# yxlao/deepSpeech

Hardware: AMD Instinct MI355X
Metric: audio-sec/sec training throughput (whole node), DS2 BiGRU (higher is better)
Workload: dtype bf16; 1 GPU; model=DeepSpeech2 2xconv(32) + 5xBiGRU-800 bidirectional + CTC, global_batch=32, seq_len=1000, parallelism=dp1, engine=hip

## Files before the change

### deepspeech_amd/csrc/api.h

```cpp
#pragma once
#include <hip/hip_runtime_api.h>
#include <stddef.h>

extern "C" {

struct DS2Fill {
  int n;
  unsigned* ptr[8];
  unsigned long long words[8];
  unsigned pattern[8];
};

hipEvent_t ds2_take_stop_event();
void ds2_arm_stop_event(hipEvent_t e);

int ds2_multi_fill(int n, void* const* ptrs, const unsigned long long* bytes, const unsigned* patterns,
                   hipStream_t st);
int ds2_multi_copy(int n, void* const* dst, const void* const* src, const unsigned long long* rows,
                   const unsigned* src_row, const unsigned* dst_row, const unsigned* src_pitch,
                   const unsigned* dst_pitch, float* sdst, const float* svals, int ns, hipStream_t st);
int ds2_wait_resident(const unsigned* word, long long timeout, hipStream_t st);
int ds2_prep_inputs(const float* x, void* y, long long n, const int* lens_in, int* lens_out, int nl,
                    hipStream_t st);
int ds2_transpose_bf16(const void* in, void* out, int R, int C, int ldi, int ldo, hipStream_t st);
// ... 205 lines not shown
                     int W, unsigned seed_lo, unsigned seed_hi, unsigned step_lo, unsigned step_hi,
                     unsigned first_utt, hipStream_t st);
int ds2_specaug_mean(const float* x, const int* lens, float* mean, int B, int T, int F, hipStream_t st);
int ds2_specaug_apply(const float* x, const int* lens, const int* plan, const float* mean, float* out, int B, int T,
                      int F, int nF, int nT, int inplace, hipStream_t st);

int ds2_seq_dropout(const void* x, void* out, const int* ctr, int T, int N, int H, unsigned seed_lo,
                    unsigned seed_hi, int site, int thr, float scale, int locked, hipStream_t st);

struct DS2Conv1WgradBn {
  const void *dz, *y1;
  const float *mean, *invstd, *gamma, *beta, *dbeta, *dgamma;
};

struct DS2Conv2DgradBn {
  const void* y1;
  const float *mean, *invstd, *gamma, *beta;
  float* part;
};

size_t ds2_conv2_fwd_smem(int F1);
size_t ds2_conv2_dgrad_smem(int F2);
size_t ds2_conv2_wgrad_smem(int F1);
long long ds2_conv2_wgrad_part_floats(int grid);
long long ds2_conv1_wgrad_part_floats(int grid);
int ds2_conv1_fwd_grid(int N, int T1);
int ds2_conv1_fwd(const void* x, const void* w, const float* bias, void* y, float* part, int N, int T, int F0,
                  int T1, int F1, hipStream_t st);
int ds2_conv2_fwd(const void* x, const void* w, const float* bias, void* y, float* part, int grid, int N, int T1,
                  int F1, int T2, int F2, long long* trace, hipStream_t st);
int ds2_conv2_dgrad(const void* dy, const void* w, void* dx, int grid, int N, int T1, int F1, int T2, int F2,
                    const DS2Conv2DgradBn* bn, long long* trace, hipStream_t st);
int ds2_conv2_wgrad(const void* dy, const void* x, float* part, int grid, float* dw, int N, int T1, int F1, int T2,
                    int F2, hipStream_t st);
int ds2_conv1_wgrad(const void* dy, const void* x, float* part, int grid, float* dw, int N, int T, int F0, int T1,
                    int F1, const DS2Conv1WgradBn* bn, hipStream_t st);
int ds2_bn_cl_finalize(const float* part, int nb, double M, float eps, float* mean, float* invstd, float* run_mean,
                       float* run_var, float momentum, hipStream_t st);
int ds2_bn_cl_apply(const void* y, const float* mean, const float* invstd, const float* gamma, const float* beta,
                    void* out, int N, int T, int F, int tmaj, hipStream_t st);
int ds2_bn_cl_bwd(const void* dz, const void* y, const float* mean, const float* invstd, const float* gamma,
                  const float* beta, float* part, int nb, float* dgamma, float* dbeta, void* dy, int N, int T, int F,
                  int tmaj, int part_ready, hipStream_t st);

struct DS2Feat {
  const void* pcm;
  long long row_stride;
  int S, lead, mode, B, T_max;
  const int* lens;
  const float* offset;
  const float* gain;
  const float* basis;
  const int* mel_idx;
  const float* mel_w;
  const float* dct;
  const float* lifter;
  void* out;
  int* frames;
};

int ds2_audio_stats(const void* pcm, int in_i16, long long row_stride, int S, int B, const int* lens, float* offset,
                    float* gain, hipStream_t st);
int ds2_featurize(const DS2Feat* a, int kind, int in_i16, int out_bf16, hipStream_t st);

}
```

### deepspeech_amd/csrc/bindings.cpp

```cpp
#include <torch/extension.h>
#include <c10/hip/HIPStream.h>
#include <hip/hip_runtime.h>

#include <cstdint>
#include <string>
#include <vector>

#include "api.h"

namespace {

using OptT = c10::optional<at::Tensor>;

hipStream_t cur_stream() { return c10::hip::getCurrentHIPStream().stream(); }

void check(int rc, const char* what) {
  TORCH_CHECK(rc == 0, "deepspeech_amd kernel launch failed in ", what, " (code ", rc, ")");
}

constexpr unsigned kLightEvent = hipEventDisableTiming;

int64_t event_new(unsigned flags) {
  hipEvent_t e = nullptr;
  TORCH_CHECK(hipEventCreateWithFlags(&e, flags ? flags : kLightEvent) == hipSuccess, "hipEventCreateWithFlags");
// ... 474 lines not shown
  need_bf16(x, "x"); need_bf16(w, "w"); need_bf16(y, "y");
  TORCH_CHECK(x.dim() == 4 && y.dim() == 4 && x.size(3) == 32 && y.size(3) == 32 && w.numel() == 32 * 32 * 50,
              "conv2_fwd shapes");
  TORCH_CHECK(grid > 0, "grid");
  need_f32(part, "part", grid * 64);
  check(ds2_conv2_fwd(x.data_ptr(), w.data_ptr(), ptr_or_null<float>(bias, "bias"), y.data_ptr(),
                      part.data_ptr<float>(), (int)grid, (int)x.size(0), (int)x.size(1), (int)x.size(2),
                      (int)y.size(1), (int)y.size(2), trace_ptr(trace), cur_stream()), "conv2_fwd");
}

void conv2_dgrad(at::Tensor dy, at::Tensor w, at::Tensor dx, int64_t grid, OptT y1, OptT mean, OptT invstd,
                 OptT gamma, OptT beta, OptT part, OptT trace) {
  need_bf16(dy, "dy"); need_bf16(w, "w"); need_bf16(dx, "dx");
  TORCH_CHECK(dy.dim() == 4 && dx.dim() == 4 && dy.size(3) == 32 && dx.size(3) == 32 && w.numel() == 32 * 32 * 50,
              "conv2_dgrad shapes");
  TORCH_CHECK(grid > 0, "grid");
  DS2Conv2DgradBn bn{};
  const bool with_bn = y1.has_value();
  if (with_bn) {
    TORCH_CHECK(mean && invstd && gamma && beta && part, "conv2_dgrad: the BN arguments come all or none");
    need_bf16(*y1, "y1");
    TORCH_CHECK(y1->sizes() == dx.sizes(), "y1 must have dx's shape");
    need_f32(*mean, "mean", 32); need_f32(*invstd, "invstd", 32); need_f32(*gamma, "gamma", 32);
    need_f32(*beta, "beta", 32); need_f32(*part, "part", grid * 64);
    bn = DS2Conv2DgradBn{y1->data_ptr(), mean->data_ptr<float>(), invstd->data_ptr<float>(),
                         gamma->data_ptr<float>(), beta->data_ptr<float>(), part->data_ptr<float>()};
  }
  check(ds2_conv2_dgrad(dy.data_ptr(), w.data_ptr(), dx.data_ptr(), (int)grid, (int)dx.size(0), (int)dx.size(1),
                        (int)dx.size(2), (int)dy.size(1), (int)dy.size(2), with_bn ? &bn : nullptr,
                        trace_ptr(trace), cur_stream()),
        "conv2_dgrad");
}

void conv2_wgrad(at::Tensor dy, at::Tensor x, at::Tensor part, at::Tensor dw, int64_t grid) {
  need_bf16(dy, "dy"); need_bf16(x, "x");
  TORCH_CHECK(grid > 0, "grid");
  need_f32(part, "part", ds2_conv2_wgrad_part_floats((int)grid));
  need_f32(dw, "dw", 32 * 32 * 50);
  check(ds2_conv2_wgrad(dy.data_ptr(), x.data_ptr(), part.data_ptr<float>(), (int)grid, dw.data_ptr<float>(),
                        (int)x.size(0), (int)x.size(1), (int)x.size(2), (int)dy.size(1), (int)dy.size(2),
                        cur_stream()), "conv2_wgrad");
}

void conv1_wgrad(at::Tensor dy, at::Tensor x, at::Tensor part, at::Tensor dw, int64_t grid, OptT y1, OptT mean,
                 OptT invstd, OptT gamma, OptT beta, OptT dbeta, OptT dgamma) {
  need_bf16(dy, "dy"); need_bf16(x, "x");
  TORCH_CHECK(grid > 0, "grid");
  need_f32(part, "part", ds2_conv1_wgrad_part_floats((int)grid));
  need_f32(dw, "dw", 32 * 100);
  DS2Conv1WgradBn bn{};
  const bool with_bn = y1.has_value();
  if (with_bn) {
    TORCH_CHECK(mean && invstd && gamma && beta && dbeta && dgamma, "conv1_wgrad: the BN arguments come all or none");
    need_bf16(*y1, "y1");
    TORCH_CHECK(y1->sizes() == dy.sizes(), "y1 must have dz's shape");
    for (const OptT* t : {&mean, &invstd, &gamma, &beta, &dbeta, &dgamma}) need_f32(**t, "bn vector", 32);
    bn = DS2Conv1WgradBn{dy.data_ptr(), y1->data_ptr(), mean->data_ptr<float>(), invstd->data_ptr<float>(),
                         gamma->data_ptr<float>(), beta->data_ptr<float>(), dbeta->data_ptr<float>(),
                         dgamma->data_ptr<float>()};
  }
  check(ds2_conv1_wgrad(with_bn ? nullptr : dy.data_ptr(), x.data_ptr(), part.data_ptr<float>(), (int)grid,
                        dw.data_ptr<float>(), (int)x.size(0), (int)x.size(1), (int)x.size(2), (int)dy.size(1),
                        (int)dy.size(2), with_bn ? &bn : nullptr, cur_stream()), "conv1_wgrad");
}
int64_t conv2_wgrad_part_floats(int64_t grid) { return ds2_conv2_wgrad_part_floats((int)grid); }
int64_t conv1_wgrad_part_floats(int64_t grid) { return ds2_conv1_wgrad_part_floats((int)grid); }

void bn_cl_finalize(at::Tensor part, int64_t nb, double M, double eps, at::Tensor mean, at::Tensor invstd,
                    OptT run_mean, OptT run_var, double momentum) {
  need_f32(part, "part", nb * 64);
  need_f32(mean, "mean", 32); need_f32(invstd, "invstd", 32);
  check(ds2_bn_cl_finalize(part.data_ptr<float>(), (int)nb, M, (float)eps, mean.data_ptr<float>(),
                           invstd.data_ptr<float>(), ptr_or_null<float>(run_mean, "run_mean"),
                           ptr_or_null<float>(run_var, "run_var"), (float)momentum, cur_stream()), "bn_cl_finalize");
// ... 875 lines not shown
        py::arg("alpha") = 1.0, py::arg("alpha_dev") = py::none(), py::arg("alpha_dev2") = py::none(),
        py::arg("a_col") = false, py::arg("b_col") = false, py::arg("splits") = 1, py::arg("ws") = py::none(),
        py::arg("cnt") = py::none(), py::arg("max_grid") = 0, py::arg("fill") = std::vector<at::Tensor>{},
        py::arg("fill_pat") = std::vector<int64_t>{}, py::arg("ext_red") = false);
  m.def("gemm8_group", &gemm8_group, py::arg("A"), py::arg("B"), py::arg("C"), py::arg("epi"), py::arg("splits"),
        py::arg("a_col"), py::arg("b_col"), py::arg("ws"), py::arg("cnt"), py::arg("max_grid"));
  m.def("gemm8_splits", [](int64_t K, bool fp8, int64_t S) { return ds2_gemm8_splits((int)K, fp8 ? 1 : 0, (int)S); });
  m.def("multi_fill", &multi_fill);
  m.def("col_sum", &col_sum);
  m.def("wait_resident", &wait_resident);
  m.def("fc_bias_grad", &fc_bias_grad);
  m.def("ctc_beam", &ctc_beam);
  m.def("ctc_beam_backtrack", &ctc_beam_backtrack);
  m.def("ctc_beam_lm", &ctc_beam_lm);
  m.def("ctc_beam_backtrack_lm", &ctc_beam_backtrack_lm);
  m.def("event_new", &event_new, py::arg("flags") = 0);
  m.def("arm_stop_event", &arm_stop_event);
  m.def("disarm_stop_event", &disarm_stop_event);
  m.def("event_free", &event_free);
  m.def("event_record", &event_record);
  m.def("event_wait", &event_wait);
  m.def("event_query", &event_query);
  m.def("stream_wait", &stream_wait);
  m.def("ctc_greedy", &ctc_greedy, py::arg("logits"), py::arg("lens"), py::arg("labels"), py::arg("counts"),
        py::arg("blank"), py::arg("score") = py::none());
  m.def("conv1_fwd", &conv1_fwd);
  m.def("conv1_fwd_grid", &conv1_fwd_grid);
  m.def("conv2_fwd", &conv2_fwd, py::arg("x"), py::arg("w"), py::arg("bias"), py::arg("y"), py::arg("part"),
        py::arg("grid"), py::arg("trace") = py::none());
  m.def("conv2_dgrad", &conv2_dgrad, py::arg("dy"), py::arg("w"), py::arg("dx"), py::arg("grid"),
        py::arg("y1") = py::none(), py::arg("mean") = py::none(), py::arg("invstd") = py::none(),
        py::arg("gamma") = py::none(), py::arg("beta") = py::none(), py::arg("part") = py::none(),
        py::arg("trace") = py::none());
  m.def("conv2_wgrad", &conv2_wgrad);
  m.def("conv1_wgrad", &conv1_wgrad, py::arg("dy"), py::arg("x"), py::arg("part"), py::arg("dw"), py::arg("grid"),
        py::arg("y1") = py::none(), py::arg("mean") = py::none(), py::arg("invstd") = py::none(),
        py::arg("gamma") = py::none(), py::arg("beta") = py::none(), py::arg("dbeta") = py::none(),
        py::arg("dgamma") = py::none());
  m.def("conv2_wgrad_part_floats", &conv2_wgrad_part_floats);
  m.def("conv1_wgrad_part_floats", &conv1_wgrad_part_floats);
  m.def("bn_cl_finalize", &bn_cl_finalize);
  m.def("bn_cl_apply", &bn_cl_apply);
  m.def("bn_cl_bwd", &bn_cl_bwd, py::arg("dz"), py::arg("y"), py::arg("mean"), py::arg("invstd"), py::arg("gamma"),
        py::arg("beta"), py::arg("part"), py::arg("nb"), py::arg("dgamma"), py::arg("dbeta"), py::arg("dy"),
        py::arg("tmaj"), py::arg("part_ready") = 0);
  m.def("gemm", &gemm, py::arg("A"), py::arg("B"), py::arg("C"), py::arg("bias"), py::arg("M"), py::arg("N"),
        py::arg("K"), py::arg("a_col"), py::arg("b_col"), py::arg("epi"), py::arg("alpha"), py::arg("cfg"),
        py::arg("alpha_dev") = py::none(), py::arg("Ml") = 0, py::arg("Nl") = 0, py::arg("Kl") = 0,
        py::arg("fill") = std::vector<at::Tensor>{}, py::arg("fill_pat") = std::vector<int64_t>{});
  m.def("gemm_tile", &gemm_tile);
  m.def("head_ctc", &head_ctc, py::arg("h"), py::arg("W"), py::arg("bias"), py::arg("lens"), py::arg("labels"),
        py::arg("label_lens"), py::arg("loss"), py::arg("G"), py::arg("ws"), py::arg("blank"), py::arg("zero_inf"),
        py::arg("mean") = py::none(), py::arg("counter") = py::none(), py::arg("first_bad") = py::none());
  m.def("fc_logits", &fc_logits);
  m.def("lookahead", &lookahead);
  m.def("lookahead_wgrad_parts", &lookahead_wgrad_parts);
  m.def("lookahead_wgrad", &lookahead_wgrad);
  m.def("lookahead_stream", &lookahead_stream);
  m.def("specaug_plan", &specaug_plan);
  m.def("specaug_mean", &specaug_mean);
  m.def("specaug_apply", &specaug_apply, py::arg("x"), py::arg("lens"), py::arg("plan"), py::arg("fill"),
        py::arg("out"), py::arg("nF"), py::arg("nT"), py::arg("inplace"));
  m.def("seq_dropout", &seq_dropout, py::arg("x"), py::arg("out"), py::arg("ctr"), py::arg("seed_lo"),
        py::arg("seed_hi"), py::arg("site"), py::arg("thr"), py::arg("scale"), py::arg("locked"));
  m.def("audio_stats", &audio_stats, py::arg("pcm"), py::arg("lens"), py::arg("offset"), py::arg("gain"));
  m.def("featurize", &featurize, py::arg("pcm"), py::arg("lens"), py::arg("offset"), py::arg("gain"),
        py::arg("basis"), py::arg("mel_idx"), py::arg("mel_w"), py::arg("dct"), py::arg("lifter"), py::arg("kind"),
// ... 13 lines not shown
```

### deepspeech_amd/csrc/conv_frontend.hip

```cpp
#include "common.h"

using namespace ds2;

namespace {

typedef __attribute__((ext_vector_type(16))) float f32x16;
typedef __attribute__((ext_vector_type(4))) short s16x4;
typedef __attribute__((address_space(3))) void lds_void_t;
typedef __attribute__((address_space(3))) s16x4 lds_s16x4_t;

constexpr int CC = 32;
constexpr float CLIP = 20.0f;
constexpr int MT = 3;

__device__ __forceinline__ f32x16 mfma32(bf16x8 a, bf16x8 b, f32x16 c) {
  return __builtin_amdgcn_mfma_f32_32x32x16_bf16(a, b, c, 0, 0, 0);
}

__device__ __forceinline__ void glds16(const void* g, void* lds_wave_base) {
  __builtin_amdgcn_global_load_lds(g, (lds_void_t*)lds_wave_base, 16, 0, 0);
}

__device__ __forceinline__ unsigned swz(unsigned R, unsigned c) { return R * 64u + ((c ^ ((R >> 2) & 3u)) << 4); }

// ... 182 lines not shown
          ssum += vb;
          ssq += vb * vb;
        }
      }
    lds_barrier();
    {
      i32x4* dst = (i32x4*)(a.y + ((size_t)n * a.T2 + t2) * a.F2 * CC);
      for (int q = tid; q < a.F2 * 4; q += 256) dst[q] = ((const i32x4*)stg)[q];
    }
    c2_stamp(a.trace, it, 4);
    lds_barrier();
    if (tile + per < t_hi) issue(tile + per);
    c2_stamp(a.trace, it, 5);
  }
  __syncthreads();
  write_stats(ssum, ssq, (float*)red, 4, a.part);
}

struct Conv2Dgrad {
  const bf16_t* dy;
  const bf16_t* w;
  bf16_t* dx;
  int N, T1, F1, T2, F2;
  const bf16_t* y1;
  const float *mean, *invstd, *gamma, *beta;
  float* part;
  long long* trace;
};
constexpr int C2D_KPW = 25;
constexpr int C2D_PR = 4 + 32 * MT;
constexpr int C2D_BUF = 5 * C2D_PR * PR;
constexpr int C2D_RED = 4 * 6 * 64 * 16;
constexpr int C2D_ROW = 80 * 64;
constexpr int C2D_SMEM = C2D_BUF + C2D_RED + 2 * C2D_ROW;
static_assert(C2D_SMEM >= 16 * CC * C2_KT * C2_KF * 2, "one co half of the weights is staged through LDS");

template <int W>
__device__ __forceinline__ void conv2_dgrad_body(const Conv2Dgrad& a);

__global__ __launch_bounds__(256) __attribute__((amdgpu_waves_per_eu(2, 2))) void conv2_dgrad_kernel(Conv2Dgrad a) {
  DS2_DCHECK(a.F2 <= 32 * MT - 4 && a.F1 == a.F2 + 4 && a.F1 > 64 && a.F1 <= 80);
  switch (uni(threadIdx.x >> 6)) {
    case 0: conv2_dgrad_body<0>(a); break;
    case 1: conv2_dgrad_body<1>(a); break;
    case 2: conv2_dgrad_body<2>(a); break;
    default: conv2_dgrad_body<3>(a); break;
  }
}

template <int W>
__device__ __forceinline__ void conv2_dgrad_body(const Conv2Dgrad& a) {
  extern __shared__ __attribute__((aligned(16))) unsigned char smem[];
  constexpr int w = W, par = W & 1, kh = W >> 1, S0 = kh * C2D_KPW;
  const int tid = threadIdx.x, lane = tid & 63;
  const int hi = lane >> 5, col = lane & 31;
  unsigned char* const buf = smem;
  f32x4* red = (f32x4*)(smem + C2D_BUF);
  unsigned short* stg = (unsigned short*)(smem + C2D_BUF + C2D_RED + par * C2D_ROW);

  bf16x8 bfr[C2D_KPW];
  {
    const unsigned short* wl = (const unsigned short*)smem;
    for (int hh = 0; hh < 2; ++hh) {
      const i32x4* src = (const i32x4*)(a.w + (size_t)hh * 16 * CC * C2_KT * C2_KF);
      for (int o = tid; o < 16 * CC * C2_KT * C2_KF / 8; o += 256) ((i32x4*)smem)[o] = src[o];
      __syncthreads();
#pragma unroll
// ... 6 lines not shown
          bfr[i][j] = (short)wl[(((8 * hi + j) * CC + col) * C2_KT + 2 * ai + par) * C2_KF + kf];
      }
      __syncthreads();
    }
  }
  for (int o = tid * 16; o < C2D_BUF; o += 256 * 16) *(i32x4*)(buf + o) = (i32x4){0, 0, 0, 0};

  const int U = (a.T1 + 1) >> 1;
  const int ntiles = a.N * U;
  const int F2 = a.F2, nq = 5 * F2;
  const int X = (gridDim.x % 8 == 0) ? 8 : 1;
  const int per = (int)gridDim.x / X, xi = (int)blockIdx.x % X, wi = (int)blockIdx.x / X;
  const int t_lo = (int)((long long)ntiles * xi / X), t_hi = (int)((long long)ntiles * (xi + 1) / X);

  auto issue = [&](int t) {
    const int n = t / U, u = t - n * U;
    const bf16_t* base = a.dy + (size_t)n * a.T2 * F2 * CC;
#pragma unroll
    for (int i = 0; i < 8; ++i) {
      const int k = w + 4 * i;
      if (k < 30) {
        const int j = k / 6, r = k % 6;
        const int q = 64 * r + lane;
        if (q < nq) {
          const int pos = (q * 52429) >> 18, c = min(q - 5 * pos, 3);
          const int row = min(max(u - 4 + j, 0), a.T2 - 1);
          glds16(base + ((size_t)row * F2 + pos) * CC + c * 8, buf + (j * C2D_PR + 4) * PR + 1024 * r);
        }
      }
    }
  };
  const unsigned char* const lbase = buf + col * PR + hi * 16;
  const bool bn = a.mean != nullptr;
  const float bmu = bn ? a.mean[col] : 0.f, bis = bn ? a.invstd[col] : 0.f;
  const float bg = bn ? a.gamma[col] : 0.f, bbt = bn ? a.beta[col] : 0.f;
  float bs = 0.f, bq = 0.f;
  auto ldA = [&](int i, bf16x8 (&dst)[MT]) {
    const int s = S0 + i;
    const int ai = s / 10, kf = (s % 10) >> 1;
    const int off = ((4 - ai) * C2D_PR + 4 - kf) * PR + (s & 1) * 32;
#pragma unroll
    for (int m = 0; m < MT; ++m) dst[m] = *(const bf16x8*)(lbase + off + m * 32 * PR);
  };

  __syncthreads();
  int it = 0;
  if (t_lo + wi < t_hi) issue(t_lo + wi);
  for (int tile = t_lo + wi; tile < t_hi; tile += per, ++it) {
    const int n = tile / U, u = tile - n * U;
    c2_stamp(a.trace, it, 0);
    asm volatile("s_waitcnt vmcnt(0)" ::: "memory");
    __syncthreads();
    c2_stamp(a.trace, it, 1);
    f32x16 acc[MT];
#pragma unroll
    for (int m = 0; m < MT; ++m) acc[m] = (f32x16){};
    bf16x8 af[2][MT];
    ldA(0, af[0]);
#pragma unroll
    for (int i = 0; i < C2D_KPW; ++i) {
      if (i + 1 < C2D_KPW) ldA(i + 1, af[(i + 1) & 1]);
      const int t2 = u - (S0 + i) / 10;
      if (t2 >= 0 && t2 < a.T2) {
#pragma unroll
        for (int m = 0; m < MT; ++m) acc[m] = mfma32(af[i & 1][m], bfr[i], acc[m]);
      }
    }
    c2_stamp(a.trace, it, 2);
    lds_barrier();
#pragma unroll
    for (int m = 0; m < MT; ++m)
#pragma unroll
      for (int j = 0; j < 2; ++j) {
        const int g = 2 * (1 - kh) + j;
        red[((w * MT + m) * 2 + j) * 64 + lane] = (f32x4){acc[m][4 * g], acc[m][4 * g + 1], acc[m][4 * g + 2], acc[m][4 * g + 3]};
      }
    lds_barrier();
    f32x4 own[MT][2];
#pragma unroll
    for (int m = 0; m < MT; ++m)
#pragma unroll
      for (int j = 0; j < 2; ++j) {
        const int g = 2 * kh + j;
        own[m][j] = (f32x4){acc[m][4 * g], acc[m][4 * g + 1], acc[m][4 * g + 2], acc[m][4 * g + 3]} +
                    red[(((w ^ 2) * MT + m) * 2 + j) * 64 + lane];
      }
    c2_stamp(a.trace, it, 3);
    const int t1 = 2 * u + par;
    const bool out = t1 < a.T1;
    const size_t rowoff = ((size_t)n * a.T1 + t1) * a.F1 * CC;
    if (out) {
      unsigned short yv[MT][2][4];
      if (bn) {
        const unsigned short* yb = (const unsigned short*)a.y1 + rowoff + 4 * hi * CC + col;
        const int lastoff = (a.F1 - 1 - 4 * hi) * CC;
#pragma unroll
        for (int m = 0; m < MT; ++m)
#pragma unroll
          for (int j = 0; j < 2; ++j)
#pragma unroll
            for (int e = 0; e < 4; ++e) {
              const int fo = (32 * m + 8 * (2 * kh + j) + e) * CC;
              yv[m][j][e] = m < 2 ? yb[fo] : yb[min(fo, lastoff)];
            }
      }
#pragma unroll
      for (int m = 0; m < MT; ++m)
#pragma unroll
        for (int j = 0; j < 2; ++j)
#pragma unroll
          for (int e = 0; e < 4; ++e) {
            const int f1 = 32 * m + 8 * (2 * kh + j) + 4 * hi + e;
            if (m < 2 || f1 < a.F1) {
              const bf16_t d = f2bf(own[m][j][e]);
              stg[f1 * CC + col] = d;
              if (bn) {
                const float xh = (bf2f(yv[m][j][e]) - bmu) * bis;
                const float zz = xh * bg + bbt;
                const float dd = (zz > 0.f && zz < CLIP) ? bf2f(d) : 0.f;
                bs += dd;
                bq += dd * xh;
              }
            }
          }
    }
    lds_barrier();
    if (out) {
      i32x4* dst = (i32x4*)(a.dx + rowoff);
      for (int q = kh * 64 + lane; q < a.F1 * 4; q += 128) dst[q] = ((const i32x4*)stg)[q];
    }
    c2_stamp(a.trace, it, 4);
    if (tile + per < t_hi) issue(tile + per);
    c2_stamp(a.trace, it, 5);
  }
  if (bn) {
    bs += __shfl_xor(bs, 32, 64);
    bq += __shfl_xor(bq, 32, 64);
    float* sh = (float*)red;
    __syncthreads();
    if (lane < 32) { sh[(w * 32 + lane) * 2] = bs; sh[(w * 32 + lane) * 2 + 1] = bq; }
    __syncthreads();
    if (tid < 64) a.part[(size_t)blockIdx.x * 64 + tid] = sh[tid] + sh[64 + tid] + sh[128 + tid] + sh[192 + tid];
  }
}

struct Conv2Wgrad {
  const bf16_t* dy;
  const bf16_t* x;
  float* part;
  int N, T1, F1, T2, F2;
};
constexpr int C2W_PAIRS = C2_KT * C2_KF;
constexpr int C2W_WAVES = 8;
constexpr int C2W_PPW = 7;

__global__ __launch_bounds__(512) void conv2_wgrad_kernel(Conv2Wgrad a) {
  extern __shared__ __attribute__((aligned(16))) unsigned char smem[];
  const int tid = threadIdx.x, lane = tid & 63, w = uni(tid >> 6);
  const int dyBytes = 80 * 64;
  const int xBytes = (9 * a.F1 + 84) * 64;
  const int bufBytes = dyBytes + xBytes;
  unsigned char* const buf0 = smem;
  unsigned char* const buf1 = smem + bufBytes;
  for (int b = 0; b < 2; ++b) {
    unsigned char* bb = b ? buf1 : buf0;
    for (int o = a.F2 * 64 + tid * 4; o < dyBytes; o += 512 * 4) *(unsigned*)(bb + o) = 0u;
    for (int o = 10 * a.F1 * 64 + tid * 4; o < xBytes; o += 512 * 4) *(unsigned*)(bb + dyBytes + o) = 0u;
  }
  const int ntiles = a.N * a.T2;
  const int dyChunks = a.F2 * 4, xChunks = 10 * a.F1 * 4;
  auto issue = [&](int t, unsigned char* dst) {
    const int n = t / a.T2, t2 = t - n * a.T2;
    const unsigned char* sdy = (const unsigned char*)(a.dy + ((size_t)n * a.T2 + t2) * a.F2 * CC);
    const unsigned char* sx = (const unsigned char*)(a.x + ((size_t)n * a.T1 + 2 * t2) * a.F1 * CC);
    for (int p0 = w * 64; p0 < dyChunks; p0 += 512) {
      const int p = p0 + lane;
      if (p < dyChunks) glds16(sdy + (size_t)p * 16, dst + (size_t)p0 * 16);
    }
    for (int p0 = w * 64; p0 < xChunks; p0 += 512) {
      const int p = p0 + lane;
      if (p < xChunks) glds16(sx + (size_t)p * 16, dst + dyBytes + (size_t)p0 * 16);
    }
  };
  const int g = lane >> 4, h = g >> 1, cb = (g & 1) * 16, q = (lane & 15) >> 2, pp = lane & 3;
  const unsigned lofs = (unsigned)((8 * h + q) * 64 + (cb + 4 * pp) * 2);
  const int npairs = (w < C2W_PAIRS - 6 * C2W_WAVES) ? 7 : 6;

  f32x16 acc[C2W_PPW];
#pragma unroll
  for (int i = 0; i < C2W_PPW; ++i) acc[i] = (f32x16){};
  __syncthreads();
  int it = 0;
  if ((int)blockIdx.x < ntiles) issue(blockIdx.x, buf0);
  for (int tile = blockIdx.x; tile < ntiles; tile += gridDim.x, ++it) {
    const unsigned char* cur = (it & 1) ? buf1 : buf0;
    asm volatile("s_waitcnt vmcnt(0)" ::: "memory");
    __syncthreads();
    if (tile + (int)gridDim.x < ntiles) issue(tile + gridDim.x, (it & 1) ? buf0 : buf1);
    const unsigned char* xs = cur + dyBytes;
#pragma unroll
    for (int kk = 0; kk < 5; ++kk) {
      const unsigned k0 = (unsigned)(16 * kk) * 64u;
      const bf16x8 av = cat8(tr_read(cur + k0 + lofs), tr_read(cur + k0 + lofs + 4 * 64));
#pragma unroll
      for (int i = 0; i < C2W_PPW; ++i) {
        if (i < npairs) {
          const int P = w + C2W_WAVES * i;
          const int kt = P / 5, kf = P - 5 * (P / 5);
          const unsigned rb = (unsigned)(kt * a.F1 + kf) * 64u + k0 + lofs;
          const bf16x8 bv = cat8(tr_read(xs + rb), tr_read(xs + rb + 4 * 64));
          acc[i] = mfma32(av, bv, acc[i]);
        }
      }
    }
  }
  f32x4* out = (f32x4*)(a.part + (size_t)blockIdx.x * C2W_PAIRS * 1024);
#pragma unroll
  for (int i = 0; i < C2W_PPW; ++i) {
    if (i < npairs) {
      const int P = w + C2W_WAVES * i;
#pragma unroll
      for (int r4 = 0; r4 < 4; ++r4)
        out[(P * 4 + r4) * 64 + lane] = (f32x4){acc[i][4 * r4], acc[i][4 * r4 + 1], acc[i][4 * r4 + 2], acc[i][4 * r4 + 3]};
    }
  }
}

template <int KIND>
__global__ __launch_bounds__(256) void wgrad_reduce_kernel(const float* __restrict__ part, int nb, int E,
                                                           float* __restrict__ dw) {
  __shared__ f32x4 sh[4][64];
  const int tid = threadIdx.x, g = tid >> 6, l = tid & 63;
  const int e4 = blockIdx.x * 64 + l, E4 = E >> 2;
  const f32x4* p4 = (const f32x4*)part;
  f32x4 s0 = {}, s1 = {};
  int b = g;
  for (; b + 4 < nb; b += 8) {
    s0 += p4[(size_t)b * E4 + e4];
    s1 += p4[(size_t)(b + 4) * E4 + e4];
  }
  if (b < nb) s0 += p4[(size_t)b * E4 + e4];
  sh[g][l] = s0 + s1;
  __syncthreads();
  if (g != 0) return;
  const f32x4 v = sh[0][l] + sh[1][l] + sh[2][l] + sh[3][l];
#pragma unroll
// ... 434 lines not shown
  const long long total = (long long)N * T * F * 4, step = (long long)gridDim.x * 256;
  const bf16x8* y8 = (const bf16x8*)y;
  const bf16x8* d8 = (const bf16x8*)dz;
  bf16x8* o8 = (bf16x8*)dy;
  long long e = (long long)blockIdx.x * 256 + tid;
  for (; e + 3 * step < total; e += 4 * step) {
    bf16x8 v[4], d[4];
#pragma unroll
    for (int k = 0; k < 4; ++k) { v[k] = y8[e + k * step]; d[k] = d8[e + k * step]; }
#pragma unroll
    for (int k = 0; k < 4; ++k) o8[e + k * step] = one(v[k], d[k]);
  }
  for (; e < total; e += step) o8[e] = one(y8[e], d8[e]);
}

template <typename K>
int set_smem(K kernel, size_t bytes) {
  return (int)hipFuncSetAttribute(reinterpret_cast<const void*>(kernel), hipFuncAttributeMaxDynamicSharedMemorySize,
                                  (int)bytes);
}

int shape_ok(int T1, int F1, int T2, int F2) {
  if (F1 < 5 || F1 > 80 || F2 != F1 - 4) return -40;
  if (T1 < 10 || T2 != (T1 - 10) / 2 + 1) return -41;
  return 0;
}

}

extern "C" {

size_t ds2_conv2_fwd_smem(int) { return (size_t)C2F_SMEM; }
size_t ds2_conv2_dgrad_smem(int) { return (size_t)C2D_SMEM; }
size_t ds2_conv2_wgrad_smem(int F1) { return (size_t)2 * (80 * 64 + (9 * F1 + 84) * 64); }
long long ds2_conv2_wgrad_part_floats(int grid) { return (long long)grid * C2W_PAIRS * 1024; }
long long ds2_conv1_wgrad_part_floats(int grid) { return (long long)grid * 5 * 1024; }
int ds2_conv1_fwd_grid(int N, int T1) { return N * ((T1 + C1_ROWS - 1) / C1_ROWS); }

int ds2_conv2_fwd(const void* x, const void* w, const float* bias, void* y, float* part, int grid, int N, int T1,
                  int F1, int T2, int F2, long long* trace, hipStream_t st) {
  if (int e = shape_ok(T1, F1, T2, F2)) return e;
  const size_t smem = ds2_conv2_fwd_smem(F1);
  DS2_HIP_CHECK((hipError_t)set_smem(conv2_fwd_kernel, smem));
  Conv2Fwd a{(const bf16_t*)x, (const bf16_t*)w, bias, (bf16_t*)y, part, N, T1, F1, T2, F2, trace};
  hipLaunchKernelGGL(conv2_fwd_kernel, dim3(grid), dim3(256), smem, st, a);
  return (int)hipGetLastError();
}

int ds2_conv2_dgrad(const void* dy, const void* w, void* dx, int grid, int N, int T1, int F1, int T2, int F2,
                    const DS2Conv2DgradBn* bn, long long* trace, hipStream_t st) {
  if (int e = shape_ok(T1, F1, T2, F2)) return e;
  if (F1 <= 64) return -42;
  const size_t smem = ds2_conv2_dgrad_smem(F2);
  DS2_HIP_CHECK((hipError_t)set_smem(conv2_dgrad_kernel, smem));
  Conv2Dgrad a{(const bf16_t*)dy, (const bf16_t*)w, (bf16_t*)dx, N, T1, F1, T2, F2,
               bn ? (const bf16_t*)bn->y1 : nullptr, bn ? bn->mean : nullptr, bn ? bn->invstd : nullptr,
               bn ? bn->gamma : nullptr, bn ? bn->beta : nullptr, bn ? bn->part : nullptr, trace};
  hipLaunchKernelGGL(conv2_dgrad_kernel, dim3(grid), dim3(256), smem, st, a);
  return (int)hipGetLastError();
}

int ds2_conv2_wgrad(const void* dy, const void* x, float* part, int grid, float* dw, int N, int T1, int F1, int T2,
                    int F2, hipStream_t st) {
  if (int e = shape_ok(T1, F1, T2, F2)) return e;
  const size_t smem = ds2_conv2_wgrad_smem(F1);
  DS2_HIP_CHECK((hipError_t)set_smem(conv2_wgrad_kernel, smem));
  Conv2Wgrad a{(const bf16_t*)dy, (const bf16_t*)x, part, N, T1, F1, T2, F2};
  hipLaunchKernelGGL(conv2_wgrad_kernel, dim3(grid), dim3(512), smem, st, a);
  hipLaunchKernelGGL(wgrad_reduce_kernel<0>, dim3(C2W_PAIRS * 1024 / 256), dim3(256), 0, st, part, grid,
                     C2W_PAIRS * 1024, dw);
  return (int)hipGetLastError();
}

int ds2_conv1_fwd(const void* x, const void* w, const float* bias, void* y, float* part, int N, int T, int F0,
                  int T1, int F1, hipStream_t st) {
  if (F1 > 96 || F1 != (F0 - 5) / 2 + 1 || T1 != (T - 20) / 2 + 1 || T1 < 1) return -42;
  Conv1Fwd a{(const bf16_t*)x, (const bf16_t*)w, bias, (bf16_t*)y, part, N, T, F0, T1, F1};
  hipLaunchKernelGGL(conv1_fwd_kernel, dim3(ds2_conv1_fwd_grid(N, T1)), dim3(256), 0, st, a);
  return (int)hipGetLastError();
}

int ds2_conv1_wgrad(const void* dy, const void* x, float* part, int grid, float* dw, int N, int T, int F0, int T1,
                    int F1, const DS2Conv1WgradBn* bn, hipStream_t st) {
  if (F1 > 80 || F1 != (F0 - 5) / 2 + 1 || T1 != (T - 20) / 2 + 1 || T1 < 1) return -43;
  if ((dy == nullptr) == (bn == nullptr)) return -44;
  DS2_HIP_CHECK((hipError_t)set_smem(conv1_wgrad_kernel, C1W_SMEM));
  Conv1Wgrad a{(const bf16_t*)dy, (const bf16_t*)x, part, N, T, F0, T1, F1,
               bn ? (const bf16_t*)bn->dz : nullptr, bn ? (const bf16_t*)bn->y1 : nullptr,
               bn ? bn->mean : nullptr, bn ? bn->invstd : nullptr, bn ? bn->gamma : nullptr,
               bn ? bn->beta : nullptr, bn ? bn->dbeta : nullptr, bn ? bn->dgamma : nullptr,
               (float)((double)N * T1 * F1)};
  hipLaunchKernelGGL(conv1_wgrad_kernel, dim3(grid), dim3(256), C1W_SMEM, st, a);
  hipLaunchKernelGGL(wgrad_reduce_kernel<1>, dim3(5 * 1024 / 256), dim3(256), 0, st, part, grid, 5 * 1024, dw);
  return (int)hipGetLastError();
}

int ds2_bn_cl_finalize(const float* part, int nb, double M, float eps, float* mean, float* invstd, float* run_mean,
                       float* run_var, float momentum, hipStream_t st) {
  hipLaunchKernelGGL(bn_cl_finalize_kernel, dim3(CC), dim3(256), 0, st, part, nb, M, eps, mean, invstd, run_mean,
                     run_var, momentum);
  return (int)hipGetLastError();
// ... 38 lines not shown
```

Before: 41860 audio-sec/sec.

## Add producer-wave ring pipeline to conv2 wgrad and vectorize dgrad BN reduction

Rewrites the conv2 weight-gradient kernel so a dedicated producer wave streams input rows into a multi-slot LDS ring. Each block works on a contiguous run of time steps, which lets it reuse overlapping input rows across neighbouring outputs instead of reloading the full 10-row window for every tile. It uses vmcnt-based partial waits to keep several loads in flight. The conv2 dgrad BN statistics are restructured: BN parameters are staged in LDS, y1 is prefetched as 16-byte vectors before the barrier, and the reduction is done on the vectorized store path with per-channel accumulators and shuffle reductions. It also adds optional tracing. The costs are more registers, a larger LDS footprint and more complex synchronization.

```diff
diff --git a/deepspeech_amd/csrc/api.h b/deepspeech_amd/csrc/api.h
--- a/deepspeech_amd/csrc/api.h
+++ b/deepspeech_amd/csrc/api.h
@@ -261,7 +261,7 @@
 int ds2_conv2_dgrad(const void* dy, const void* w, void* dx, int grid, int N, int T1, int F1, int T2, int F2,
                     const DS2Conv2DgradBn* bn, long long* trace, hipStream_t st);
 int ds2_conv2_wgrad(const void* dy, const void* x, float* part, int grid, float* dw, int N, int T1, int F1, int T2,
-                    int F2, hipStream_t st);
+                    int F2, long long* trace, hipStream_t st);
 int ds2_conv1_wgrad(const void* dy, const void* x, float* part, int grid, float* dw, int N, int T, int F0, int T1,
                     int F1, const DS2Conv1WgradBn* bn, hipStream_t st);
 int ds2_bn_cl_finalize(const float* part, int nb, double M, float eps, float* mean, float* invstd, float* run_mean,
diff --git a/deepspeech_amd/csrc/bindings.cpp b/deepspeech_amd/csrc/bindings.cpp
--- a/deepspeech_amd/csrc/bindings.cpp
+++ b/deepspeech_amd/csrc/bindings.cpp
@@ -530,14 +530,14 @@
         "conv2_dgrad");
 }
 
-void conv2_wgrad(at::Tensor dy, at::Tensor x, at::Tensor part, at::Tensor dw, int64_t grid) {
+void conv2_wgrad(at::Tensor dy, at::Tensor x, at::Tensor part, at::Tensor dw, int64_t grid, OptT trace) {
   need_bf16(dy, "dy"); need_bf16(x, "x");
   TORCH_CHECK(grid > 0, "grid");
   need_f32(part, "part", ds2_conv2_wgrad_part_floats((int)grid));
   need_f32(dw, "dw", 32 * 32 * 50);
   check(ds2_conv2_wgrad(dy.data_ptr(), x.data_ptr(), part.data_ptr<float>(), (int)grid, dw.data_ptr<float>(),
                         (int)x.size(0), (int)x.size(1), (int)x.size(2), (int)dy.size(1), (int)dy.size(2),
-                        cur_stream()), "conv2_wgrad");
+                        trace_ptr(trace), cur_stream()), "conv2_wgrad");
 }
 
 void conv1_wgrad(at::Tensor dy, at::Tensor x, at::Tensor part, at::Tensor dw, int64_t grid, OptT y1, OptT mean,
@@ -1479,7 +1479,8 @@
         py::arg("y1") = py::none(), py::arg("mean") = py::none(), py::arg("invstd") = py::none(),
         py::arg("gamma") = py::none(), py::arg("beta") = py::none(), py::arg("part") = py::none(),
         py::arg("trace") = py::none());
-  m.def("conv2_wgrad", &conv2_wgrad);
+  m.def("conv2_wgrad", &conv2_wgrad, py::arg("dy"), py::arg("x"), py::arg("part"), py::arg("dw"), py::arg("grid"),
+        py::arg("trace") = py::none());
   m.def("conv1_wgrad", &conv1_wgrad, py::arg("dy"), py::arg("x"), py::arg("part"), py::arg("dw"), py::arg("grid"),
         py::arg("y1") = py::none(), py::arg("mean") = py::none(), py::arg("invstd") = py::none(),
         py::arg("gamma") = py::none(), py::arg("beta") = py::none(), py::arg("dbeta") = py::none(),
diff --git a/deepspeech_amd/csrc/conv_frontend.hip b/deepspeech_amd/csrc/conv_frontend.hip
--- a/deepspeech_amd/csrc/conv_frontend.hip
+++ b/deepspeech_amd/csrc/conv_frontend.hip
@@ -238,7 +238,9 @@
 constexpr int C2D_BUF = 5 * C2D_PR * PR;
 constexpr int C2D_RED = 4 * 6 * 64 * 16;
 constexpr int C2D_ROW = 80 * 64;
-constexpr int C2D_SMEM = C2D_BUF + C2D_RED + 2 * C2D_ROW;
+constexpr int C2D_BNP = 4 * CC * 4;
+constexpr int C2D_SMEM = C2D_BUF + C2D_RED + 2 * C2D_ROW + C2D_BNP;
+static_assert(2 * C2D_SMEM <= 160 * 1024, "two workgroups per CU");
 static_assert(C2D_SMEM >= 16 * CC * C2_KT * C2_KF * 2, "one co half of the weights is staged through LDS");
 
 template <int W>
@@ -311,9 +313,15 @@
   };
   const unsigned char* const lbase = buf + col * PR + hi * 16;
   const bool bn = a.mean != nullptr;
-  const float bmu = bn ? a.mean[col] : 0.f, bis = bn ? a.invstd[col] : 0.f;
-  const float bg = bn ? a.gamma[col] : 0.f, bbt = bn ? a.beta[col] : 0.f;
-  float bs = 0.f, bq = 0.f;
+  float bs[8], bq[8];
+#pragma unroll
+  for (int j = 0; j < 8; ++j) bs[j] = bq[j] = 0.f;
+  float* const bnp = (float*)(smem + C2D_BUF + C2D_RED + 2 * C2D_ROW);
+  if (bn && tid < 128) {
+    const float* src = tid < 32 ? a.mean : tid < 64 ? a.invstd : tid < 96 ? a.gamma : a.beta;
+    bnp[tid] = src[tid & 31];
+  }
+  const int nchunk = a.F1 * 4;
   auto ldA = [&](int i, bf16x8 (&dst)[MT]) {
     const int s = S0 + i;
     const int ai = s / 10, kf = (s % 10) >> 1;
@@ -331,6 +339,9 @@
     asm volatile("s_waitcnt vmcnt(0)" ::: "memory");
     __syncthreads();
     c2_stamp(a.trace, it, 1);
+    const int t1 = 2 * u + par;
+    const bool out = t1 < a.T1;
+    const size_t rowoff = ((size_t)n * a.T1 + t1) * a.F1 * CC;
     f32x16 acc[MT];
 #pragma unroll
     for (int m = 0; m < MT; ++m) acc[m] = (f32x16){};
@@ -346,6 +357,13 @@
       }
     }
     c2_stamp(a.trace, it, 2);
+    i32x4 yv[3] = {};
+    if (bn) {
+      const i32x4* ysrc = (const i32x4*)(a.y1 + ((size_t)n * a.T1 + min(t1, a.T1 - 1)) * a.F1 * CC);
+#pragma unroll
+      for (int i = 0; i < 3; ++i)
+        if (i < 2 || kh == 0) yv[i] = ysrc[min(kh * 64 + lane + 128 * i, nchunk - 1)];
+    }
     lds_barrier();
 #pragma unroll
     for (int m = 0; m < MT; ++m)
@@ -365,24 +383,7 @@
                     red[(((w ^ 2) * MT + m) * 2 + j) * 64 + lane];
       }
     c2_stamp(a.trace, it, 3);
-    const int t1 = 2 * u + par;
-    const bool out = t1 < a.T1;
-    const size_t rowoff = ((size_t)n * a.T1 + t1) * a.F1 * CC;
     if (out) {
-      unsigned short yv[MT][2][4];
-      if (bn) {
-        const unsigned short* yb = (const unsigned short*)a.y1 + rowoff + 4 * hi * CC + col;
-        const int lastoff = (a.F1 - 1 - 4 * hi) * CC;
-#pragma unroll
-        for (int m = 0; m < MT; ++m)
-#pragma unroll
-          for (int j = 0; j < 2; ++j)
-#pragma unroll
-            for (int e = 0; e < 4; ++e) {
-              const int fo = (32 * m + 8 * (2 * kh + j) + e) * CC;
-              yv[m][j][e] = m < 2 ? yb[fo] : yb[min(fo, lastoff)];
-            }
-      }
 #pragma unroll
       for (int m = 0; m < MT; ++m)
 #pragma unroll
@@ -390,34 +391,62 @@
 #pragma unroll
           for (int e = 0; e < 4; ++e) {
             const int f1 = 32 * m + 8 * (2 * kh + j) + 4 * hi + e;
-            if (m < 2 || f1 < a.F1) {
-              const bf16_t d = f2bf(own[m][j][e]);
-              stg[f1 * CC + col] = d;
-              if (bn) {
-                const float xh = (bf2f(yv[m][j][e]) - bmu) * bis;
-                const float zz = xh * bg + bbt;
-                const float dd = (zz > 0.f && zz < CLIP) ? bf2f(d) : 0.f;
-                bs += dd;
-                bq += dd * xh;
-              }
-            }
+            if (m < 2 || f1 < a.F1) stg[f1 * CC + col] = f2bf(own[m][j][e]);
           }
     }
     lds_barrier();
     if (out) {
       i32x4* dst = (i32x4*)(a.dx + rowoff);
-      for (int q = kh * 64 + lane; q < a.F1 * 4; q += 128) dst[q] = ((const i32x4*)stg)[q];
+#pragma unroll
+      for (int i = 0; i < 3; ++i) {
+        const int q = kh * 64 + lane + 128 * i;
+        if (i < 2 || (kh == 0 && q < nchunk)) {
+          const i32x4 dv = ((const i32x4*)stg)[q];
+          dst[q] = dv;
+          if (bn) {
+            const f32x4* pv = (const f32x4*)bnp + 2 * (lane & 3);
+            const f32x4 mu0 = pv[0], mu1 = pv[1], is0 = pv[8], is1 = pv[9];
+            const f32x4 g0 = pv[16], g1 = pv[17], b0 = pv[24], b1 = pv[25];
+            const float bmu[8] = {mu0[0], mu0[1], mu0[2], mu0[3], mu1[0], mu1[1], mu1[2], mu1[3]};
+            const float bis[8] = {is0[0], is0[1], is0[2], is0[3], is1[0], is1[1], is1[2], is1[3]};
+            const float bg[8] = {g0[0], g0[1], g0[2], g0[3], g1[0], g1[1], g1[2], g1[3]};
+            const float bbt[8] = {b0[0], b0[1], b0[2], b0[3], b1[0], b1[1], b1[2], b1[3]};
+#pragma unroll
+            for (int j = 0; j < 8; ++j) {
+              const unsigned dw = (unsigned)dv[j >> 1], yw = (unsigned)yv[i][j >> 1];
+              const float d = __uint_as_float((j & 1) ? (dw & 0xffff0000u) : (dw << 16));
+              const float y = __uint_as_float((j & 1) ? (yw & 0xffff0000u) : (yw << 16));
+              const float xh = (y - bmu[j]) * bis[j];
+              const float zz = xh * bg[j] + bbt[j];
+              const float dd = (zz > 0.f && zz < CLIP) ? d : 0.f;
+              bs[j] += dd;
+              bq[j] += dd * xh;
+            }
+          }
+        }
+      }
     }
     c2_stamp(a.trace, it, 4);
     if (tile + per < t_hi) issue(tile + per);
     c2_stamp(a.trace, it, 5);
   }
   if (bn) {
-    bs += __shfl_xor(bs, 32, 64);
-    bq += __shfl_xor(bq, 32, 64);
+#pragma unroll
+    for (int j = 0; j < 8; ++j)
+#pragma unroll
+      for (int o = 4; o < 64; o <<= 1) {
+        bs[j] += __shfl_xor(bs[j], o, 64);
+        bq[j] += __shfl_xor(bq[j], o, 64);
+      }
     float* sh = (float*)red;
     __syncthreads();
-    if (lane < 32) { sh[(w * 32 + lane) * 2] = bs; sh[(w * 32 + lane) * 2 + 1] = bq; }
+    if (lane < 4) {
+#pragma unroll
+      for (int j = 0; j < 8; ++j) {
+        sh[(w * 32 + 8 * lane + j) * 2] = bs[j];
+        sh[(w * 32 + 8 * lane + j) * 2 + 1] = bq[j];
+      }
+    }
     __syncthreads();
     if (tid < 64) a.part[(size_t)blockIdx.x * 64 + tid] = sh[tid] + sh[64 + tid] + sh[128 + tid] + sh[192 + tid];
   }
@@ -428,39 +457,59 @@
   const bf16_t* x;
   float* part;
   int N, T1, F1, T2, F2;
+  long long* trace;
 };
 constexpr int C2W_PAIRS = C2_KT * C2_KF;
 constexpr int C2W_WAVES = 8;
 constexpr int C2W_PPW = 7;
-
-__global__ __launch_bounds__(512) void conv2_wgrad_kernel(Conv2Wgrad a) {
+#ifndef DS2_C2W_D
+#define DS2_C2W_D 3
+#endif
+constexpr int C2W_D = DS2_C2W_D;
+constexpr int C2W_R = C2_KT + 2 * C2W_D;
+constexpr int C2W_RD = 1 + C2W_D;
+constexpr int C2W_XS = 84 * 64;
+constexpr int C2W_DS = 80 * 64;
+constexpr int C2W_SMEM = C2W_R * C2W_XS + C2W_RD * C2W_DS;
+constexpr int C2W_THREADS = (C2W_WAVES + 1) * 64;
+static_assert(C2W_D >= 1 && 15 * (C2W_D - 1) <= 63, "vmcnt is a 6-bit counter");
+static_assert(C2W_SMEM <= 160 * 1024, "one workgroup per CU");
+
+struct C2WUnit {
+  int tile, t2, s;
+  __device__ __forceinline__ void next(int T2) {
+    if (s < 4) { ++s; return; }
+    ++tile;
+    if (++t2 == T2) { t2 = 0; s = 0; } else s = 4;
+  }
+};
+
+template <int N>
+__device__ __forceinline__ void c2w_wait() { asm volatile("s_waitcnt vmcnt(%0)" ::"n"(N) : "memory"); }
+__device__ __forceinline__ void c2w_wait_units(int J) {
+  switch (J) {
+#define C2W_CASE(j) case j: c2w_wait<j * (C2W_D - 1)>(); break;
+    C2W_CASE(3) C2W_CASE(4) C2W_CASE(5) C2W_CASE(6) C2W_CASE(7) C2W_CASE(8) C2W_CASE(9) C2W_CASE(10)
+    C2W_CASE(11) C2W_CASE(12) C2W_CASE(13) C2W_CASE(14) C2W_CASE(15)
+#undef C2W_CASE
+    default: c2w_wait<0>(); break;
+  }
+}
+__device__ __forceinline__ void c2w_stamp(long long* tr, int unit, int k) {
+  if (tr != nullptr && blockIdx.x < 8 && threadIdx.x == 0 && unit < 16)
+    tr[((int)blockIdx.x * 16 + unit) * C2_TRACE + k] = __builtin_amdgcn_s_memrealtime();
+}
+
+__global__ __launch_bounds__(C2W_THREADS) void conv2_wgrad_kernel(Conv2Wgrad a) {
   extern __shared__ __attribute__((aligned(16))) unsigned char smem[];
   const int tid = threadIdx.x, lane = tid & 63, w = uni(tid >> 6);
-  const int dyBytes = 80 * 64;
-  const int xBytes = (9 * a.F1 + 84) * 64;
-  const int bufBytes = dyBytes + xBytes;
-  unsigned char* const buf0 = smem;
-  unsigned char* const buf1 = smem + bufBytes;
-  for (int b = 0; b < 2; ++b) {
-    unsigned char* bb = b ? buf1 : buf0;
-    for (int o = a.F2 * 64 + tid * 4; o < dyBytes; o += 512 * 4) *(unsigned*)(bb + o) = 0u;
-    for (int o = 10 * a.F1 * 64 + tid * 4; o < xBytes; o += 512 * 4) *(unsigned*)(bb + dyBytes + o) = 0u;
-  }
-  const int ntiles = a.N * a.T2;
-  const int dyChunks = a.F2 * 4, xChunks = 10 * a.F1 * 4;
-  auto issue = [&](int t, unsigned char* dst) {
-    const int n = t / a.T2, t2 = t - n * a.T2;
-    const unsigned char* sdy = (const unsigned char*)(a.dy + ((size_t)n * a.T2 + t2) * a.F2 * CC);
-    const unsigned char* sx = (const unsigned char*)(a.x + ((size_t)n * a.T1 + 2 * t2) * a.F1 * CC);
-    for (int p0 = w * 64; p0 < dyChunks; p0 += 512) {
-      const int p = p0 + lane;
-      if (p < dyChunks) glds16(sdy + (size_t)p * 16, dst + (size_t)p0 * 16);
-    }
-    for (int p0 = w * 64; p0 < xChunks; p0 += 512) {
-      const int p = p0 + lane;
-      if (p < xChunks) glds16(sx + (size_t)p * 16, dst + dyBytes + (size_t)p0 * 16);
-    }
-  };
+  unsigned char* const zring = smem;
+  unsigned char* const dring = smem + C2W_R * C2W_XS;
+  for (int o = tid * 16; o < C2W_SMEM; o += C2W_THREADS * 16) *(i32x4*)(smem + o) = (i32x4){0, 0, 0, 0};
+  const int ntiles = a.N * a.T2, T2 = a.T2;
+  const int G = (int)gridDim.x, X = (G % 8 == 0) ? 8 : 1;
+  const int run = ((int)blockIdx.x % X) * (G / X) + (int)blockIdx.x / X;
+  const int lo = (int)((long long)ntiles * run / G), hi = (int)((long long)ntiles * (run + 1) / G);
   const int g = lane >> 4, h = g >> 1, cb = (g & 1) * 16, q = (lane & 15) >> 2, pp = lane & 3;
   const unsigned lofs = (unsigned)((8 * h + q) * 64 + (cb + 4 * pp) * 2);
   const int npairs = (w < C2W_PAIRS - 6 * C2W_WAVES) ? 7 : 6;
@@ -469,28 +518,76 @@
 #pragma unroll
   for (int i = 0; i < C2W_PPW; ++i) acc[i] = (f32x16){};
   __syncthreads();
-  int it = 0;
-  if ((int)blockIdx.x < ntiles) issue(blockIdx.x, buf0);
-  for (int tile = blockIdx.x; tile < ntiles; tile += gridDim.x, ++it) {
-    const unsigned char* cur = (it & 1) ? buf1 : buf0;
-    asm volatile("s_waitcnt vmcnt(0)" ::: "memory");
-    __syncthreads();
-    if (tile + (int)gridDim.x < ntiles) issue(tile + gridDim.x, (it & 1) ? buf0 : buf1);
-    const unsigned char* xs = cur + dyBytes;
-#pragma unroll
-    for (int kk = 0; kk < 5; ++kk) {
-      const unsigned k0 = (unsigned)(16 * kk) * 64u;
-      const bf16x8 av = cat8(tr_read(cur + k0 + lofs), tr_read(cur + k0 + lofs + 4 * 64));
-#pragma unroll
-      for (int i = 0; i < C2W_PPW; ++i) {
-        if (i < npairs) {
+  if (w == C2W_WAVES) {
+    const int dyChunks = a.F2 * 4, xChunks = a.F1 * 4;
+    const int J = 2 * ((xChunks + 63) >> 6) + ((dyChunks + 63) >> 6);
+    C2WUnit pf{lo, lo % T2, 0};
+    int zs = 0, ds = 0;
+    auto issue = [&]() {
+      const int n = pf.tile / T2;
+      const unsigned char* sdy = (const unsigned char*)(a.dy + (size_t)pf.tile * a.F2 * CC);
+      const unsigned char* sx = (const unsigned char*)(a.x + ((size_t)n * a.T1 + 2 * pf.t2 + 2 * pf.s) * a.F1 * CC);
+      for (int j = 0; j < 2; ++j) {
+        unsigned char* dst = zring + (zs + j) * C2W_XS;
+        for (int p0 = 0; p0 < xChunks; p0 += 64) {
+          const int p = p0 + lane;
+          if (p < xChunks) glds16(sx + ((size_t)j * xChunks + p) * 16, dst + p0 * 16);
+        }
+      }
+      for (int p0 = 0; p0 < dyChunks; p0 += 64) {
+        const int p = p0 + lane;
+        if (p < dyChunks) glds16(sdy + (size_t)p * 16, dring + ds * C2W_DS + p0 * 16);
+      }
+      zs = (zs + 2 == C2W_R) ? 0 : zs + 2;
+      ds = (ds + 1 == C2W_RD) ? 0 : ds + 1;
+      C2WUnit nx = pf;
+      nx.next(T2);
+      if (nx.tile < hi) pf = nx;
+    };
+    if (lo < hi) {
+      for (int d = 0; d < C2W_D; ++d) issue();
+      for (C2WUnit cu{lo, lo % T2, 0}; cu.tile < hi; cu.next(T2)) {
+        c2w_wait_units(J);
+        __builtin_amdgcn_s_barrier();
+        issue();
+      }
+      c2w_wait<0>();
+    }
+    return;
+  }
+  {
+    int zh = C2W_R - 8, ds = 0, k = 0;
+    for (C2WUnit cu{lo, lo % T2, 0}; cu.tile < hi; cu.next(T2), ++k) {
+      c2w_stamp(a.trace, k, 0);
+      lds_barrier();
+      c2w_stamp(a.trace, k, 1);
+      if (cu.s == 4) {
+        const unsigned char* cur = dring + ds * C2W_DS + lofs;
+        const unsigned char* xs[C2W_PPW];
+#pragma unroll
+        for (int i = 0; i < C2W_PPW; ++i) {
           const int P = w + C2W_WAVES * i;
-          const int kt = P / 5, kf = P - 5 * (P / 5);
-          const unsigned rb = (unsigned)(kt * a.F1 + kf) * 64u + k0 + lofs;
-          const bf16x8 bv = cat8(tr_read(xs + rb), tr_read(xs + rb + 4 * 64));
-          acc[i] = mfma32(av, bv, acc[i]);
+          const int kt = P / 5, kf = P - 5 * kt;
+          int sl = zh + kt;
+          sl = sl >= C2W_R ? sl - C2W_R : sl;
+          xs[i] = zring + sl * C2W_XS + kf * 64 + lofs;
         }
-      }
+#pragma unroll
+        for (int kk = 0; kk < 5; ++kk) {
+          const unsigned k0 = (unsigned)(16 * kk) * 64u;
+          const bf16x8 av = cat8(tr_read(cur + k0), tr_read(cur + k0 + 4 * 64));
+#pragma unroll
+          for (int i = 0; i < C2W_PPW; ++i) {
+            if (i < npairs) {
+              const bf16x8 bv = cat8(tr_read(xs[i] + k0), tr_read(xs[i] + k0 + 4 * 64));
+              acc[i] = mfma32(av, bv, acc[i]);
+            }
+          }
+        }
+        c2w_stamp(a.trace, k, 2);
+      }
+      zh = (zh + 2 >= C2W_R) ? zh + 2 - C2W_R : zh + 2;
+      ds = (ds + 1 == C2W_RD) ? 0 : ds + 1;
     }
   }
   f32x4* out = (f32x4*)(a.part + (size_t)blockIdx.x * C2W_PAIRS * 1024);
@@ -991,7 +1088,7 @@
 
 size_t ds2_conv2_fwd_smem(int) { return (size_t)C2F_SMEM; }
 size_t ds2_conv2_dgrad_smem(int) { return (size_t)C2D_SMEM; }
-size_t ds2_conv2_wgrad_smem(int F1) { return (size_t)2 * (80 * 64 + (9 * F1 + 84) * 64); }
+size_t ds2_conv2_wgrad_smem(int) { return (size_t)C2W_SMEM; }
 long long ds2_conv2_wgrad_part_floats(int grid) { return (long long)grid * C2W_PAIRS * 1024; }
 long long ds2_conv1_wgrad_part_floats(int grid) { return (long long)grid * 5 * 1024; }
 int ds2_conv1_fwd_grid(int N, int T1) { return N * ((T1 + C1_ROWS - 1) / C1_ROWS); }
@@ -1020,12 +1117,12 @@
 }
 
 int ds2_conv2_wgrad(const void* dy, const void* x, float* part, int grid, float* dw, int N, int T1, int F1, int T2,
-                    int F2, hipStream_t st) {
+                    int F2, long long* trace, hipStream_t st) {
   if (int e = shape_ok(T1, F1, T2, F2)) return e;
   const size_t smem = ds2_conv2_wgrad_smem(F1);
   DS2_HIP_CHECK((hipError_t)set_smem(conv2_wgrad_kernel, smem));
-  Conv2Wgrad a{(const bf16_t*)dy, (const bf16_t*)x, part, N, T1, F1, T2, F2};
-  hipLaunchKernelGGL(conv2_wgrad_kernel, dim3(grid), dim3(512), smem, st, a);
+  Conv2Wgrad a{(const bf16_t*)dy, (const bf16_t*)x, part, N, T1, F1, T2, F2, trace};
+  hipLaunchKernelGGL(conv2_wgrad_kernel, dim3(grid), dim3(C2W_THREADS), smem, st, a);
   hipLaunchKernelGGL(wgrad_reduce_kernel<0>, dim3(C2W_PAIRS * 1024 / 256), dim3(256), 0, st, part, grid,
                      C2W_PAIRS * 1024, dw);
   return (int)hipGetLastError();
```

After: 42130 audio-sec/sec, median of 6. Within noise of the previous version (+0.6%).
